# ruiminshen/yolo2-pytorch

Measured on AMD Instinct MI355X. Metric: images/sec (416x416) train+detect, Darknet-19 YOLOv2: value = TRAIN step, batch 64 per GPU (configs[2]) at every N; detect (configs[1]) = roofline.detect_images_per_sec, higher is better.
Workload: dtype f32; 1 GPU; Darknet-19 YOLOv2 20-class train 416x416 batch-64/GPU: fwd + region loss + bwd + SGD (BASELINE configs[2]); classes=20, global_batch=64, parallelism=single GPU, weights=random-init seed 0 (bench_data.randomize)

## Files before the change

yolo2-pytorch_amd/csrc/conv_wgrad.hip:

```cpp
#include <stdlib.h>
#include "common.h"

#ifndef Y2_WGRAD_SPREAD
#define Y2_WGRAD_SPREAD 1
#endif

namespace {

constexpr int NT = 256;
constexpr int KS = 32;

struct WgradArgs {
    const float* x;
    const float* dz;
    float* dw;
    float* partial;
    int B, H, W, Cin, ldx, Cout, ldz, taps;
    int Hi, Wi, stride, pad, KW;
    int M, tiles_i, tiles_j, splits, slabs_per_split;
    unsigned x_bytes, dz_bytes;
    int groups;
    long long gx, gz, gw;
    const int32_t* tile_pix;
    int zW;
};

template <int TI, int WAVES_I, int TJ = 128, bool LIN = false, bool DZRAW = false>
__global__ __launch_bounds__(NT) void conv_wgrad_kernel(const WgradArgs a) {
    constexpr unsigned OOB = 0x80000000u;
    constexpr int WAVES_J = 4 / WAVES_I;
    constexpr int WI = TI / WAVES_I, WJ = TJ / WAVES_J;
    constexpr int IB = WI / 32, JB = WJ / 32;
    constexpr int CA = TI / 4;
    constexpr int RA = NT / CA;
    constexpr int PA = KS / RA;
    constexpr int CB = TJ / 4, RB = NT / CB, PB = KS / RB;
    static_assert(WJ >= 32 && WI >= 32, "a wave owns at least one 32x32 block");
    constexpr int STAGE = KS * TI + KS * TJ;
    typedef __attribute__((address_space(3))) void* lds_ptr_t;
    extern __shared__ __attribute__((aligned(16))) float smem[];

    const int t = threadIdx.x;
    const int lane = t & 63;
    const int wave = __builtin_amdgcn_readfirstlane(t >> 6);
    const int wm = wave / WAVES_J, wn = wave % WAVES_J;
    const int l31 = lane & 31, half = lane >> 5;

    int bid = blockIdx.x;
    int grp = 0;
    if (a.groups > 1) {
        const int per = a.tiles_i * a.tiles_j * a.splits;
        grp = bid / per;
        bid -= grp * per;
    }
    const float* gx_ptr = a.x + (size_t)grp * a.gx;
    const float* gz_ptr = a.dz + (size_t)grp * a.gz;
    float* gw_ptr = a.dw + (size_t)grp * a.gw;
    const int split = bid % a.splits; bid /= a.splits;
    const int tj = bid % a.tiles_j;
    const int ti = bid / a.tiles_j;
    const int i0 = ti * TI, j0 = tj * TJ;
    const int ncols = a.taps * a.Cin;

    const int slab_lo = split * a.slabs_per_split;
    const int nslab_total = (a.M + KS - 1) / KS;
    const int slab_hi = min(nslab_total, slab_lo + a.slabs_per_split);
    const int nk = slab_hi - slab_lo;
    if (nk <= 0) return;

    const int chunk = t % CB;
    const int prow = t / CB;
    const int chunk_a = t % CA;
    const int prow_a = t / CA;
    const int ca = i0 + 4 * chunk_a;
    const bool a_ok = ca < a.Cout;
    const int jb = j0 + 4 * chunk;
    const bool b_ok = jb < ncols;
    const int tap = b_ok ? jb / a.Cin : 0;
    const int ci = b_ok ? jb - tap * a.Cin : 0;
    const int dy = tap / a.KW - a.pad;
    const int dx = tap % a.KW - a.pad;
    int pb[PB], py[PB], px[PB];
    const int q32 = KS / a.W, r32 = KS % a.W;
#pragma unroll
    for (int p = 0; p < PB; ++p) {
        const int m = slab_lo * KS + prow + RB * p;
        pb[p] = m / (a.H * a.W);
        const int idx = m - pb[p] * (a.H * a.W);
        py[p] = idx / a.W;
        px[p] = idx - py[p] * a.W;
    }
    const __amdgpu_buffer_rsrc_t rx = __builtin_amdgcn_make_buffer_rsrc(const_cast<float*>(gx_ptr), 0, a.x_bytes, 0x00020000);
    const __amdgpu_buffer_rsrc_t rz = __builtin_amdgcn_make_buffer_rsrc(const_cast<float*>(gz_ptr), 0, a.dz_bytes, 0x00020000);

    auto issue_slab = [&](int slab, int buf) {
        float* sa = smem + buf * STAGE + wave * 256;
        float* sb = smem + buf * STAGE + KS * TI + wave * 256;
#pragma unroll
        for (int p = 0; p < PA; ++p) {
            const int m = slab * KS + prow_a + RA * p;
            const unsigned va = (m < a.M && a_ok) ? (unsigned)(((size_t)m * a.ldz + ca) * 4) : OOB;
            __builtin_amdgcn_raw_ptr_buffer_load_lds(rz, (lds_ptr_t)(sa + p * RA * TI), 16, (int)va, 0, 0, 0);
        }
#pragma unroll
        for (int p = 0; p < PB; ++p) {
            const int m = slab * KS + prow + RB * p;
            const bool mok = m < a.M;
            const int yi = py[p] * a.stride + dy, xi = px[p] * a.stride + dx;
            const bool in = (unsigned)yi < (unsigned)a.Hi && (unsigned)xi < (unsigned)a.Wi;
            const unsigned vb = (mok && b_ok && in) ? (unsigned)(((size_t)((pb[p] * a.Hi + yi) * a.Wi + xi) * a.ldx + ci) * 4) : OOB;
            __builtin_amdgcn_raw_ptr_buffer_load_lds(rx, (lds_ptr_t)(sb + p * RB * TJ), 16, (int)vb, 0, 0, 0);
        }
#pragma unroll
        for (int p = 0; p < PB; ++p) {
            px[p] += r32; py[p] += q32;
            if (px[p] >= a.W) { px[p] -= a.W; py[p] += 1; }
            while (py[p] >= a.H) { py[p] -= a.H; pb[p] += 1; }
        }
    };

    const int xi = grp >> 2, nu = grp & 3;
    const bool two_i = xi == 1 || xi == 2, two_j = nu == 1 || nu == 2;
    const int i_first = xi == 3 ? 1 : 0, j_first = nu == 3 ? 1 : 0;
    const unsigned pixb = (unsigned)a.ldz * 4u;
    int e_next[PA];
    f32x4 dpx[PA][2][2];
    auto dz_table = [&](int slab) {
#pragma unroll
        for (int p = 0; p < PA; ++p) {
            const int m = slab * KS + prow_a + RA * p;
            e_next[p] = m < a.M ? a.tile_pix[m] : 0x3fffffff;
        }
    };
    auto dz_loads = [&]() {
#pragma unroll
        for (int p = 0; p < PA; ++p) {
            const int e = e_next[p];
            const unsigned pix = (unsigned)e & 0x3fffffffu;
            const bool rowok = a_ok && pix != 0x3fffffffu;
            const bool y1 = (e & 0x40000000) != 0, x1 = e < 0;
            const unsigned base = pix * pixb + (unsigned)ca * 4u;
#pragma unroll
            for (int i = 0; i < 2; ++i)
#pragma unroll
                for (int j = 0; j < 2; ++j) {
                    if ((i == 1 && !two_i) || (j == 1 && !two_j)) continue;
                    const int ii = i_first + i, jj = j_first + j;
                    const bool ok = rowok && (ii == 0 || y1) && (jj == 0 || x1);
                    dpx[p][i][j] = __builtin_bit_cast(f32x4, __builtin_amdgcn_raw_buffer_load_b128(rz, (int)(ok ? base : OOB), (ii * a.zW + jj) * (int)pixb, 0));
                }
        }
    };
    auto dz_store = [&](int buf) {
#pragma unroll
        for (int p = 0; p < PA; ++p) {
            f32x4 sj[2];
#pragma unroll
            for (int j = 0; j < 2; ++j) {
                if (j == 1 && !two_j) continue;
                sj[j] = xi == 0 ? dpx[p][0][j] : (xi == 1 ? dpx[p][0][j] + dpx[p][1][j] : (xi == 2 ? dpx[p][0][j] - dpx[p][1][j] : -dpx[p][0][j]));
            }
            const f32x4 r = nu == 0 ? sj[0] : (nu == 1 ? sj[0] + sj[1] : (nu == 2 ? sj[0] - sj[1] : -sj[0]));
            *reinterpret_cast<f32x4*>(smem + buf * STAGE + p * RA * TI + t * 4) = r;
        }
    };

    f32x16 acc[IB][JB];
#pragma unroll
    for (int i = 0; i < IB; ++i)
#pragma unroll
        for (int j = 0; j < JB; ++j)
#pragma unroll
            for (int r = 0; r < 16; ++r) acc[i][j][r] = 0.f;

    const int fa = wm * WI + l31 + half * TI;
    const int fb = KS * TI + wn * WJ + l31 + half * TJ;

    unsigned nva[PA], nvb[PB];
    if (LIN) {
#pragma unroll
        for (int p = 0; p < PA; ++p) nva[p] = a_ok ? (unsigned)(((size_t)(slab_lo * KS + prow_a + RA * p) * a.ldz + ca) * 4) : OOB;
#pragma unroll
        for (int p = 0; p < PB; ++p) nvb[p] = b_ok ? (unsigned)(((size_t)(slab_lo * KS + prow + RB * p) * a.ldx + ci) * 4) : OOB;
    }
    const unsigned step_a = a_ok ? (unsigned)(KS * a.ldz * 4) : 0u, step_b = b_ok ? (unsigned)(KS * a.ldx * 4) : 0u;
    auto plan_slab = [&](int slab) {
        if (LIN) {
#pragma unroll
            for (int p = 0; p < PA; ++p) nva[p] += step_a;
#pragma unroll
            for (int p = 0; p < PB; ++p) nvb[p] += step_b;
            return;
        }
#pragma unroll
        for (int p = 0; p < PA; ++p) {
            const int m = slab * KS + prow_a + RA * p;
            nva[p] = (m < a.M && a_ok) ? (unsigned)(((size_t)m * a.ldz + ca) * 4) : OOB;
        }
#pragma unroll
        for (int p = 0; p < PB; ++p) {
            const int m = slab * KS + prow + RB * p;
            const bool mok = m < a.M;
            const int yi = py[p] * a.stride + dy, xi = px[p] * a.stride + dx;
            const bool in = (unsigned)yi < (unsigned)a.Hi && (unsigned)xi < (unsigned)a.Wi;
            nvb[p] = (mok && b_ok && in) ? (unsigned)(((size_t)((pb[p] * a.Hi + yi) * a.Wi + xi) * a.ldx + ci) * 4) : OOB;
            px[p] += r32; py[p] += q32;
            if (px[p] >= a.W) { px[p] -= a.W; py[p] += 1; }
            while (py[p] >= a.H) { py[p] -= a.H; pb[p] += 1; }
        }
    };
    auto issue_piece = [&](int buf, int j) {
        if (j < PA) { if (!DZRAW) __builtin_amdgcn_raw_ptr_buffer_load_lds(rz, (lds_ptr_t)(smem + buf * STAGE + wave * 256 + j * RA * TI), 16, (int)nva[j], 0, 0, 0); }
        else __builtin_amdgcn_raw_ptr_buffer_load_lds(rx, (lds_ptr_t)(smem + buf * STAGE + KS * TI + wave * 256 + (j - PA) * RB * TJ), 16, (int)nvb[j - PA], 0, 0, 0);
    };
    auto compute_slab_spread = [&](int buf, int nbuf, int next_slab = 0) {
        const volatile __attribute__((address_space(3))) float* sbuf = (const volatile __attribute__((address_space(3))) float*)(smem + buf * STAGE);
        constexpr int TOTAL = (KS / 2) * IB * JB, NPIECES = PA + PB;
        constexpr int EVERY = (TOTAL / 2) / NPIECES > 0 ? (TOTAL / 2) / NPIECES : 1;
        int cnt = 0;
        float av[2][IB], bv[2][JB];
#pragma unroll
        for (int i = 0; i < IB; ++i) av[0][i] = sbuf[fa + 32 * i];
#pragma unroll
        for (int j = 0; j < JB; ++j) bv[0][j] = sbuf[fb + 32 * j];
#pragma unroll
        for (int s = 0; s < KS / 2; ++s) {
            if (s + 1 < KS / 2) {
#pragma unroll
                for (int i = 0; i < IB; ++i) av[(s + 1) & 1][i] = sbuf[fa + (s + 1) * 2 * TI + 32 * i];
#pragma unroll
                for (int j = 0; j < JB; ++j) bv[(s + 1) & 1][j] = sbuf[fb + (s + 1) * 2 * TJ + 32 * j];
            }
#pragma unroll
            for (int i = 0; i < IB; ++i)
#pragma unroll
                for (int j = 0; j < JB; ++j) {
                    acc[i][j] = __builtin_amdgcn_mfma_f32_32x32x2f32(av[s & 1][i], bv[s & 1][j], acc[i][j], 0, 0, 0);
                    if (cnt % EVERY == 0 && cnt / EVERY < NPIECES) {
                        issue_piece(nbuf, cnt / EVERY);
                        __builtin_amdgcn_sched_barrier(0);
                    }
                    if (DZRAW) {
                        if (cnt == 0) { dz_loads(); __builtin_amdgcn_sched_barrier(0); }
                        if (cnt == 2) { dz_table(next_slab + 1); __builtin_amdgcn_sched_barrier(0); }
                        if (cnt == (TOTAL * 3) / 4) { dz_store(nbuf); __builtin_amdgcn_sched_barrier(0); }
                    }
                    ++cnt;
                }
        }
#pragma unroll
        for (int j = (TOTAL + EVERY - 1) / EVERY; j < NPIECES; ++j) issue_piece(nbuf, j);
    };

    bool blk_ok[IB][JB];
    bool all_ok = true;
#pragma unroll
    for (int i = 0; i < IB; ++i)
#pragma unroll
        for (int j = 0; j < JB; ++j) {
            blk_ok[i][j] = (i0 + wm * WI + i * 32) < a.Cout && (j0 + wn * WJ + j * 32) < ncols;
            all_ok = all_ok && blk_ok[i][j];
        }
    auto compute_slab_checked = [&](int buf) {
        const float* sbuf = smem + buf * STAGE;
#pragma unroll
        for (int s = 0; s < KS / 2; ++s) {
            float av[IB], bv[JB];
#pragma unroll
            for (int i = 0; i < IB; ++i) av[i] = sbuf[fa + s * 2 * TI + 32 * i];
#pragma unroll
            for (int j = 0; j < JB; ++j) bv[j] = sbuf[fb + s * 2 * TJ + 32 * j];
#pragma unroll
            for (int i = 0; i < IB; ++i)
#pragma unroll
                for (int j = 0; j < JB; ++j)
                    if (blk_ok[i][j]) acc[i][j] = __builtin_amdgcn_mfma_f32_32x32x2f32(av[i], bv[j], acc[i][j], 0, 0, 0);
        }
    };

    auto compute_slab = [&](int buf) {
        const float* sbuf = smem + buf * STAGE;
#pragma unroll
        for (int s = 0; s < KS / 2; ++s) {
            float av[IB], bv[JB];
#pragma unroll
            for (int i = 0; i < IB; ++i) av[i] = sbuf[fa + s * 2 * TI + 32 * i];
#pragma unroll
            for (int j = 0; j < JB; ++j) bv[j] = sbuf[fb + s * 2 * TJ + 32 * j];
#pragma unroll
            for (int i = 0; i < IB; ++i)
#pragma unroll
                for (int j = 0; j < JB; ++j)
                    acc[i][j] = __builtin_amdgcn_mfma_f32_32x32x2f32(av[i], bv[j], acc[i][j], 0, 0, 0);
        }
    };

    if (DZRAW) {
        dz_table(slab_lo);
        dz_loads();
        dz_table(slab_lo + 1);
        dz_store(0);
#pragma unroll
        for (int j = PA; j < PA + PB; ++j) issue_piece(0, j);
        for (int ks = 0; ks < nk - 1; ++ks) {
            plan_slab(slab_lo + ks + 1);
            asm volatile("s_waitcnt vmcnt(0)" ::: "memory");
            __syncthreads();
            compute_slab_spread(ks & 1, (ks + 1) & 1, slab_lo + ks + 1);
        }
        asm volatile("s_waitcnt vmcnt(0)" ::: "memory");
        __syncthreads();
        compute_slab((nk - 1) & 1);
    } else {
    issue_slab(slab_lo, 0);
    if (!all_ok) {
        for (int ks = 0; ks < nk - 1; ++ks) {
            asm volatile("s_waitcnt vmcnt(0)" ::: "memory");
            __syncthreads();
            issue_slab(slab_lo + ks + 1, (ks + 1) & 1);
            compute_slab_checked(ks & 1);
        }
        asm volatile("s_waitcnt vmcnt(0)" ::: "memory");
        __syncthreads();
        compute_slab_checked((nk - 1) & 1);
    } else {
        for (int ks = 0; ks < nk - 1; ++ks) {
            if (Y2_WGRAD_SPREAD) plan_slab(slab_lo + ks + 1);
            asm volatile("s_waitcnt vmcnt(0)" ::: "memory");
            __syncthreads();
            if (Y2_WGRAD_SPREAD) {
                compute_slab_spread(ks & 1, (ks + 1) & 1);
            } else {
                issue_slab(slab_lo + ks + 1, (ks + 1) & 1);
                compute_slab(ks & 1);
            }
        }
        asm volatile("s_waitcnt vmcnt(0)" ::: "memory");
        __syncthreads();
        compute_slab((nk - 1) & 1);
    }
    }

#pragma unroll
    for (int jbk = 0; jbk < JB; ++jbk) {
        const int j = j0 + wn * WJ + jbk * 32 + l31;
        if (j >= ncols) continue;
#pragma unroll
        for (int ib = 0; ib < IB; ++ib) {
#pragma unroll
            for (int r = 0; r < 16; ++r) {
                const int co = i0 + wm * WI + ib * 32 + (r & 3) + 8 * (r >> 2) + 4 * half;
                if (co < a.Cout) {
                    if (a.partial != nullptr) {
                        a.partial[((size_t)(grp * a.splits + split) * a.Cout + co) * ncols + j] = acc[ib][jbk][r];
                        continue;
                    }
                    float* dst = gw_ptr + (size_t)co * ncols + j;
                    if (a.splits > 1) atomicAdd(dst, acc[ib][jbk][r]);
                    else *dst = acc[ib][jbk][r];
                }
            }
        }
    }
}

}

static int wgrad_tj(int ncols, int Cout) {
    if (Cout <= 32) return 128;
    const long long p128 = (long long)y2_cdiv(ncols, 128) * 128, p64 = (long long)y2_cdiv(ncols, 64) * 64;
    return (p128 * 100 >= p64 * 115) ? 64 : 128;
}

static int wgrad_splits(long long M, int ncols, int Cout, int groups, int* slabs_per_split) {
    const int TI = Cout <= 32 ? 32 : (Cout <= 64 ? 64 : 128);
    const int TJ = wgrad_tj(ncols, Cout);
    const long long tiles = (long long)y2_cdiv(Cout, TI) * y2_cdiv(ncols, TJ);
    const int slabs = y2_cdiv(M, KS);
    static const int fill_env = getenv("Y2_WGRAD_FILL") != nullptr ? atoi(getenv("Y2_WGRAD_FILL")) : 0;
    const int fill = fill_env > 0 ? fill_env : (TI * TJ >= 128 * 128 ? 2 : (TI * TJ >= 128 * 64 ? 3 : 4));
    int splits = y2_cdiv(fill * Y2_NUM_CU, tiles * groups);
    const int max_splits = slabs / 8 > 0 ? slabs / 8 : 1;
    if (splits > max_splits) splits = max_splits;
    if (splits < 1) splits = 1;
    const int sps = y2_cdiv(slabs, splits);
    if (slabs_per_split != nullptr) *slabs_per_split = sps;
    return y2_cdiv(slabs, sps);
}

int y2_internal_wgrad_needs_zero(long long M, int Cin, int Cout, int groups) {
    return (wgrad_splits(M, Cin, Cout, groups, nullptr) > 1 && !y2_det.on) ? 1 : 0;
}

struct WgradRawDz { const int32_t* tile_pix; int zW, ldz; unsigned long long bytes; };

static int wgrad_impl(const float* x, const float* dz, float* dw, int B, int Hi, int Wi, int Cin, int ldx, int Cout, int ldz,
                      int ksize, int stride, int pad, y2_stream_t stream, int groups, long long gx, long long gz, long long gw, const WgradRawDz* raw = nullptr) {
    if (!x || !dz || !dw || B <= 0 || Hi <= 0 || Wi <= 0 || Cin <= 0 || Cout <= 0) return Y2_EINVAL;
    if (ksize < 1 || ksize > 7 || stride < 1 || pad < 0) return Y2_ENOSUP;
    if (ldx < Cin || ldz < Cout) return Y2_EINVAL;
    if ((Cin & 3) || (ldx & 3) || (Cout & 3) || (ldz & 3) || !y2_aligned16(x) || !y2_aligned16(dz)) return Y2_EALIGN;
    const int H = (Hi + 2 * pad - ksize) / stride + 1, W = (Wi + 2 * pad - ksize) / stride + 1;
    if (H <= 0 || W <= 0) return Y2_EINVAL;
    const long long M = (long long)B * H * W;
    const unsigned long long xb = (unsigned long long)B * Hi * Wi * ldx * 4ull, zb = (unsigned long long)M * ldz * 4ull;
    if (M > 0x3fffffffLL || xb >= 0x7fffffffull || zb >= 0x7fffffffull) return Y2_ENOSUP;
    WgradArgs a;
    a.x = x; a.dz = dz; a.dw = dw;
    a.B = B; a.H = H; a.W = W; a.Cin = Cin; a.ldx = ldx; a.Cout = Cout; a.ldz = ldz; a.taps = ksize * ksize;
    a.Hi = Hi; a.Wi = Wi; a.stride = stride; a.pad = pad; a.KW = ksize;
    a.M = (int)M;
    a.groups = groups; a.gx = gx; a.gz = gz; a.gw = gw;
    const int TI = Cout <= 32 ? 32 : (Cout <= 64 ? 64 : 128);
    a.tiles_i = y2_cdiv(Cout, TI);
    const int TJ = wgrad_tj(a.taps * Cin, Cout);
    a.tiles_j = y2_cdiv(a.taps * Cin, TJ);
    const int tiles = a.tiles_i * a.tiles_j;
    const int slabs = y2_cdiv(M, KS);
    a.splits = wgrad_splits(M, a.taps * Cin, Cout, groups, &a.slabs_per_split);
    a.x_bytes = (unsigned)xb; a.dz_bytes = (unsigned)zb;
    a.tile_pix = nullptr; a.zW = 0;
    if (raw != nullptr) {
        if (groups != 16 || raw->bytes >= 0x7fffffffull || (raw->ldz & 3) || raw->ldz < Cout) return Y2_ENOSUP;
        a.tile_pix = raw->tile_pix; a.zW = raw->zW; a.ldz = raw->ldz; a.dz_bytes = (unsigned)raw->bytes; a.gz = 0;
    }
    a.partial = nullptr;
    const long long wsize = (long long)Cout * a.taps * Cin;
    if (y2_det.on && a.splits > 1) {
        if ((size_t)groups * a.splits * wsize * sizeof(float) > y2_det.bytes) return Y2_EINVAL;
        a.partial = y2_det.ws;
    }
    const long long grid = (long long)tiles * a.splits * groups;
    if (grid > 0x7fffffffLL) return Y2_EINVAL;
    hipStream_t s = y2_s(stream);
    const size_t lds = 2u * (size_t)(KS * TI + KS * TJ) * sizeof(float);
    const bool lin = ksize == 1 && stride == 1 && pad == 0;
#define Y2_WGRAD_LAUNCH_(TI_, WI_, TJ_, LIN_)                                                                             \
    do {                                                                                                                  \
        static Y2LdsAttr attr;                                                                                            \
        if (const int rc_ = attr.ensure(reinterpret_cast<const void*>(conv_wgrad_kernel<TI_, WI_, TJ_, LIN_>))) return rc_;     \
        Y2_LAUNCH(a.groups > 1 ? "conv_wgrad_kernel[grouped]" : "conv_wgrad_kernel", 2.0 * (double)a.M * a.Cout * a.taps * a.Cin * (a.groups > 1 ? a.groups : 1), (conv_wgrad_kernel<TI_, WI_, TJ_, LIN_>), dim3((unsigned)grid), dim3(NT), lds, s, a);                 \
    } while (0)
#define Y2_WGRAD_LAUNCH_RAW(TI_, WI_, TJ_)                                                                                \
    do {                                                                                                                  \
        static Y2LdsAttr attr;                                                                                            \
        if (const int rc_ = attr.ensure(reinterpret_cast<const void*>(conv_wgrad_kernel<TI_, WI_, TJ_, true, true>))) return rc_;     \
        Y2_LAUNCH("conv_wgrad_kernel[grouped,dz]", 2.0 * (double)a.M * a.Cout * a.taps * a.Cin * a.groups, (conv_wgrad_kernel<TI_, WI_, TJ_, true, true>), dim3((unsigned)grid), dim3(NT), lds, s, a);                 \
    } while (0)
#define Y2_WGRAD_LAUNCH(TI_, WI_, TJ_)                                                                                    \
    do {                                                                                                                  \
        if (raw != nullptr) Y2_WGRAD_LAUNCH_RAW(TI_, WI_, TJ_);                                                           \
        else if (lin) Y2_WGRAD_LAUNCH_(TI_, WI_, TJ_, true); else Y2_WGRAD_LAUNCH_(TI_, WI_, TJ_, false);                 \
    } while (0)
    if (TI == 32) Y2_WGRAD_LAUNCH(32, 1, 128);
    else if (TI == 64 && TJ == 64) Y2_WGRAD_LAUNCH(64, 2, 64);
    else if (TI == 64) Y2_WGRAD_LAUNCH(64, 1, 128);
    else if (TJ == 64) Y2_WGRAD_LAUNCH(128, 2, 64);
    else Y2_WGRAD_LAUNCH(128, 2, 128);
#undef Y2_WGRAD_LAUNCH
#undef Y2_WGRAD_LAUNCH_RAW
#undef Y2_WGRAD_LAUNCH_
    Y2_LAUNCH_CHECK();
    if (a.partial != nullptr) {
        for (int g = 0; g < groups; ++g) {
            const int rc = y2_det_reduce_f32(a.partial + (size_t)g * a.splits * wsize, a.splits, wsize, wsize, nullptr, dw + (size_t)g * gw, s);
            if (rc != Y2_OK) return rc;
        }
    }
    return Y2_OK;
}

namespace {

struct W0Args {
    const float* x; const float* dz; float* dw;
    float* partial;
    int B, H, W, Cin, Cout, ldz, rows_total;
};

template <int IB>
__global__ __launch_bounds__(256) void conv0_wgrad_kernel(const W0Args a) {
    __shared__ float red[4][IB * 32 * 33];
    const int t = threadIdx.x, lane = t & 63, wave = t >> 6;
    const int l31 = lane & 31, half = lane >> 5;
    const int K = a.Cin * 9;
    const bool jok = l31 < K;
    const int c = jok ? l31 / 9 : 0;
    const int ky = jok ? (l31 % 9) / 3 : 0, kx = jok ? l31 % 3 : 0;
    f32x16 acc[IB];
#pragma unroll
    for (int i = 0; i < IB; ++i)
#pragma unroll
        for (int r = 0; r < 16; ++r) acc[i][r] = 0.f;
    const int wid = blockIdx.x * 4 + wave, nw = gridDim.x * 4;
    for (int row = wid; row < a.rows_total; row += nw) {
        const int b = row / a.H, y = row - b * a.H;
        const int yy = y + ky - 1;
        const bool yok = jok && (unsigned)yy < (unsigned)a.H;
        const float* xr = a.x + (((size_t)b * a.Cin + c) * a.H + (yok ? yy : 0)) * a.W;
        const float* zr = a.dz + (size_t)row * a.W * a.ldz;
        for (int x0 = 0; x0 < a.W; x0 += 16) {
            float av[IB][8], bv[8];
#pragma unroll
            for (int s = 0; s < 8; ++s) {
                const int px = x0 + 2 * s + half;
                const bool pok = px < a.W;
#pragma unroll
                for (int i = 0; i < IB; ++i) {
                    const int co = i * 32 + l31;
                    av[i][s] = (pok && co < a.Cout) ? zr[(size_t)px * a.ldz + co] : 0.f;
                }
                const int xx = px + kx - 1;
                bv[s] = (pok && yok && (unsigned)xx < (unsigned)a.W) ? xr[xx] : 0.f;
            }
#pragma unroll
            for (int s = 0; s < 8; ++s)
#pragma unroll
                for (int i = 0; i < IB; ++i)
                    acc[i] = __builtin_amdgcn_mfma_f32_32x32x2f32(av[i][s], bv[s], acc[i], 0, 0, 0);
        }
    }
#pragma unroll
    for (int i = 0; i < IB; ++i)
#pragma unroll
        for (int r = 0; r < 16; ++r) {
            const int co = i * 32 + (r & 3) + 8 * (r >> 2) + 4 * half;
            red[wave][co * 33 + l31] = acc[i][r];
        }
    __syncthreads();
    for (int e = t; e < IB * 32 * 32; e += 256) {
        const int co = e >> 5, j = e & 31;
        if (co < a.Cout && j < K) {
            const float v = red[0][co * 33 + j] + red[1][co * 33 + j] + red[2][co * 33 + j] + red[3][co * 33 + j];
            if (a.partial != nullptr) a.partial[(size_t)blockIdx.x * a.Cout * K + (size_t)co * K + j] = v;
            else atomicAdd(a.dw + (size_t)co * K + j, v);
        }
    }
}

}

namespace {

struct W0FArgs {
    const float* x; const float* z; const float* scale; const float* shift; const float* mean; const float* invstd; const float* gamma;
    const float* dy_pool; const double* sums; float* dw;
    float* partial;
    int B, H, W, Cin, Cout, ldz, ldp, pairs_total, has_bn;
    unsigned z_bytes, p_bytes;
    float slope;
    double n;
};

template <int IB>
__global__ __launch_bounds__(256) void conv0_wgrad_fused_kernel(const W0FArgs a) {
    __shared__ float red[4][IB * 32 * 33];
    const int t = threadIdx.x, lane = t & 63, wave = t >> 6;
    const int l31 = lane & 31, half = lane >> 5;
    const int K = a.Cin * 9;
    const bool jok = l31 < K;
    const int c = jok ? l31 / 9 : 0;
    const int ky = jok ? (l31 % 9) / 3 : 0, kx = jok ? l31 % 3 : 0;
    float sc[IB], sh[IB], mu[IB], is[IB], gs[IB], ma[IB], mb[IB];
    bool cok[IB];
#pragma unroll
    for (int i = 0; i < IB; ++i) {
        const int co = i * 32 + l31;
        cok[i] = co < a.Cout;
        const int cc = cok[i] ? co : 0;
        sc[i] = a.scale ? a.scale[cc] : 1.f; sh[i] = a.shift ? a.shift[cc] : 0.f;
        mu[i] = a.has_bn ? a.mean[cc] : 0.f; is[i] = a.has_bn ? a.invstd[cc] : 1.f;
        if (a.has_bn == 1) { gs[i] = a.gamma[cc] * is[i]; ma[i] = (float)(a.sums[cc] / a.n); mb[i] = (float)(a.sums[a.Cout + cc] / a.n); }
        else if (a.has_bn == 2) { gs[i] = a.gamma[cc] * is[i]; ma[i] = 0.f; mb[i] = 0.f; }
        else { gs[i] = 1.f; ma[i] = 0.f; mb[i] = 0.f; }
    }
    f32x16 acc[IB];
#pragma unroll
    for (int i = 0; i < IB; ++i)
#pragma unroll
        for (int r = 0; r < 16; ++r) acc[i][r] = 0.f;
    const int wid = blockIdx.x * 4 + wave, nw = gridDim.x * 4;
    const int Hh = a.H >> 1, Wh = a.W >> 1;
    const __amdgpu_buffer_rsrc_t rz = __builtin_amdgcn_make_buffer_rsrc(const_cast<float*>(a.z), 0, a.z_bytes, 0x00020000);
    const __amdgpu_buffer_rsrc_t rp = __builtin_amdgcn_make_buffer_rsrc(const_cast<float*>(a.dy_pool), 0, a.p_bytes, 0x00020000);
    for (int pair = wid; pair < a.pairs_total; pair += nw) {
        const int b = pair / Hh, r = pair - b * Hh;
        const int y0 = 2 * r;
        const int yy0 = y0 + ky - 1, yy1 = yy0 + 1;
        const bool yok0 = jok && (unsigned)yy0 < (unsigned)a.H, yok1 = jok && (unsigned)yy1 < (unsigned)a.H;
        const float* xr0 = a.x + (((size_t)b * a.Cin + c) * a.H + (yok0 ? yy0 : 0)) * a.W;
        const float* xr1 = a.x + (((size_t)b * a.Cin + c) * a.H + (yok1 ? yy1 : 0)) * a.W;
        const unsigned zrow = (unsigned)(((size_t)(b * a.H + y0) * a.W + half) * a.ldz * 4u) + (unsigned)l31 * 4u;
        const unsigned prow = (unsigned)(((size_t)(b * Hh + r) * Wh) * a.ldp * 4u) + (unsigned)l31 * 4u;
        const unsigned zstep = 2u * (unsigned)a.ldz * 4u, z1off = (unsigned)a.W * (unsigned)a.ldz * 4u, pstep = (unsigned)a.ldp * 4u;
        for (int x0 = 0; x0 < a.W; x0 += 16) {
            float z0[IB][8], z1[IB][8], dp[IB][8], bv0[8], bv1[8];
            const unsigned zb = zrow + (unsigned)x0 * (unsigned)a.ldz * 4u, pb = prow + (unsigned)(x0 >> 1) * pstep;
#pragma unroll
            for (int s = 0; s < 8; ++s) {
                const int px = x0 + 2 * s + half;
#pragma unroll
                for (int i = 0; i < IB; ++i) {
                    z0[i][s] = __builtin_bit_cast(float, __builtin_amdgcn_raw_buffer_load_b32(rz, (int)(zb + i * 128u), (int)(s * zstep), 0));
                    z1[i][s] = __builtin_bit_cast(float, __builtin_amdgcn_raw_buffer_load_b32(rz, (int)(zb + i * 128u), (int)(s * zstep + z1off), 0));
                    dp[i][s] = __builtin_bit_cast(float, __builtin_amdgcn_raw_buffer_load_b32(rp, (int)(pb + i * 128u), (int)(s * pstep), 0));
                }
                const int xx = px + kx - 1;
                const bool xok = (unsigned)xx < (unsigned)a.W;
                bv0[s] = (xok && yok0) ? xr0[xx] : 0.f;
                bv1[s] = (xok && yok1) ? xr1[xx] : 0.f;
            }
#pragma unroll
            for (int s = 0; s < 8; ++s)
#pragma unroll
                for (int i = 0; i < IB; ++i) {
                    const float u0 = z0[i][s] * sc[i] + sh[i], u1 = z1[i][s] * sc[i] + sh[i];
                    const float v0 = u0 > 0.f ? u0 : u0 * a.slope, v1 = u1 > 0.f ? u1 : u1 * a.slope;
                    const float o0 = __shfl_xor(v0, 32), o1 = __shfl_xor(v1, 32);
                    const float q0 = half ? o0 : v0, q1 = half ? v0 : o0, q2 = half ? o1 : v1, q3 = half ? v1 : o1;
                    float best = q0; int arg = 0;
                    if (q1 > best) { best = q1; arg = 1; }
                    if (q2 > best) { best = q2; arg = 2; }
                    if (q3 > best) { best = q3; arg = 3; }
                    const float g0 = (arg == half) ? dp[i][s] : 0.f, g1 = (arg == 2 + half) ? dp[i][s] : 0.f;
                    const float ge0 = g0 * (u0 > 0.f ? 1.f : a.slope), ge1 = g1 * (u1 > 0.f ? 1.f : a.slope);
                    const float zh0 = (z0[i][s] - mu[i]) * is[i], zh1 = (z1[i][s] - mu[i]) * is[i];
                    const bool ok = (x0 + 2 * s + half) < a.W && cok[i];
                    const float d0 = ok ? gs[i] * (ge0 - ma[i] - zh0 * mb[i]) : 0.f;
                    const float d1 = ok ? gs[i] * (ge1 - ma[i] - zh1 * mb[i]) : 0.f;
                    acc[i] = __builtin_amdgcn_mfma_f32_32x32x2f32(d0, bv0[s], acc[i], 0, 0, 0);
                    acc[i] = __builtin_amdgcn_mfma_f32_32x32x2f32(d1, bv1[s], acc[i], 0, 0, 0);
                }
        }
    }
#pragma unroll
    for (int i = 0; i < IB; ++i)
#pragma unroll
        for (int r = 0; r < 16; ++r) {
            const int co = i * 32 + (r & 3) + 8 * (r >> 2) + 4 * half;
            red[wave][co * 33 + l31] = acc[i][r];
        }
    __syncthreads();
    for (int e = t; e < IB * 32 * 32; e += 256) {
        const int co = e >> 5, j = e & 31;
        if (co < a.Cout && j < K) {
            const float v = red[0][co * 33 + j] + red[1][co * 33 + j] + red[2][co * 33 + j] + red[3][co * 33 + j];
            if (a.partial != nullptr) a.partial[(size_t)blockIdx.x * a.Cout * K + (size_t)co * K + j] = v;
            else atomicAdd(a.dw + (size_t)co * K + j, v);
        }
    }
}

}

extern "C" int y2_conv0_wgrad_fused(const float* x_nchw, const float* z, const float* scale, const float* shift, const float* mean, const float* invstd,
                                    const float* gamma, float slope, const float* dy_pool, int ldp, const double* sums, float* dw,
                                    int B, int H, int W, int Cin, int Cout, int ldz, int has_bn, y2_stream_t stream) {
    if (!x_nchw || !z || !dy_pool || !dw || B <= 0 || H <= 0 || W <= 0 || Cout <= 0 || ldz < Cout || ldp < Cout) return Y2_EINVAL;
    if (has_bn < 0 || has_bn > 2 || (has_bn && (!mean || !invstd || !gamma)) || (has_bn == 1 && !sums)) return Y2_EINVAL;
    if ((H & 1) || (W & 1)) return Y2_EINVAL;
    if (Cin < 1 || Cin > 3 || Cout > 64 || (W & 15)) return Y2_ENOSUP;
    const unsigned long long zb = (unsigned long long)B * H * W * ldz * 4ull, pb = (unsigned long long)B * (H / 2) * (W / 2) * ldp * 4ull;
    if (zb >= 0xffff0000ull) return Y2_ENOSUP;
    W0FArgs a;
    a.z_bytes = (unsigned)zb; a.p_bytes = (unsigned)pb;
    a.x = x_nchw; a.z = z; a.scale = scale; a.shift = shift; a.mean = mean; a.invstd = invstd; a.gamma = gamma; a.dy_pool = dy_pool; a.sums = sums; a.dw = dw;
    a.B = B; a.H = H; a.W = W; a.Cin = Cin; a.Cout = Cout; a.ldz = ldz; a.ldp = ldp; a.pairs_total = B * (H / 2); a.has_bn = has_bn; a.slope = slope;
    a.n = (double)B * H * W;
    const int grid = a.pairs_total < 4 * 4 * Y2_NUM_CU ? y2_cdiv(a.pairs_total, 4) : 4 * Y2_NUM_CU;
    a.partial = nullptr;
    if (y2_det.on) {
        if ((size_t)grid * Cout * Cin * 9 * sizeof(float) > y2_det.bytes) return Y2_EINVAL;
        a.partial = y2_det.ws;
    }
    const double flops = 2.0 * (double)B * H * W * 9 * Cin * Cout;
    if (Cout <= 32) Y2_LAUNCH("conv0_wgrad_fused_kernel", flops, (conv0_wgrad_fused_kernel<1>), dim3(grid), dim3(256), 0, y2_s(stream), a);
    else Y2_LAUNCH("conv0_wgrad_fused_kernel", flops, (conv0_wgrad_fused_kernel<2>), dim3(grid), dim3(256), 0, y2_s(stream), a);
    Y2_LAUNCH_CHECK();
    if (a.partial != nullptr) return y2_det_reduce_f32(a.partial, grid, (long long)Cout * Cin * 9, (long long)Cout * Cin * 9, nullptr, dw, y2_s(stream));
    return Y2_OK;
}

extern "C" int y2_conv0_wgrad(const float* x_nchw, const float* dz, float* dw, int B, int H, int W, int Cin, int Cout, int ldz, y2_stream_t stream) {
    if (!x_nchw || !dz || !dw || B <= 0 || H <= 0 || W <= 0 || Cout <= 0 || ldz < Cout) return Y2_EINVAL;
    if (Cin < 1 || Cin > 3 || Cout > 64) return Y2_ENOSUP;
    W0Args a;
    a.x = x_nchw; a.dz = dz; a.dw = dw; a.B = B; a.H = H; a.W = W; a.Cin = Cin; a.Cout = Cout; a.ldz = ldz; a.rows_total = B * H;
    const int grid = a.rows_total < 4 * 4 * Y2_NUM_CU ? y2_cdiv(a.rows_total, 4) : 4 * Y2_NUM_CU;
    a.partial = nullptr;
    if (y2_det.on) {
        if ((size_t)grid * Cout * Cin * 9 * sizeof(float) > y2_det.bytes) return Y2_EINVAL;
        a.partial = y2_det.ws;
    }
    if (Cout <= 32) Y2_LAUNCH("conv0_wgrad_kernel", 2.0 * (double)B * H * W * 9 * Cin * Cout, (conv0_wgrad_kernel<1>), dim3(grid), dim3(256), 0, y2_s(stream), a);
    else Y2_LAUNCH("conv0_wgrad_kernel", 2.0 * (double)B * H * W * 9 * Cin * Cout, (conv0_wgrad_kernel<2>), dim3(grid), dim3(256), 0, y2_s(stream), a);
    Y2_LAUNCH_CHECK();
    if (a.partial != nullptr) return y2_det_reduce_f32(a.partial, grid, (long long)Cout * Cin * 9, (long long)Cout * Cin * 9, nullptr, dw, y2_s(stream));
    return Y2_OK;
}

extern "C" int y2_conv_wgrad_ex(const float* x, const float* dz, float* dw, int B, int Hi, int Wi, int Cin, int ldx, int Cout, int ldz,
                                int ksize, int stride, int pad, y2_stream_t stream) {
    return wgrad_impl(x, dz, dw, B, Hi, Wi, Cin, ldx, Cout, ldz, ksize, stride, pad, stream, 1, 0, 0, 0);
}

int y2_internal_wgrad_grouped(const float* x, const float* dz, float* dw, long long M, int Cin, int Cout, int groups, long long gx, long long gz,
                              long long gw, y2_stream_t stream) {
    if (M <= 0 || M > 0x7fffffffLL || groups < 1) return Y2_EINVAL;
    return wgrad_impl(x, dz, dw, 1, 1, (int)M, Cin, Cin, Cout, Cout, 1, 1, 0, stream, groups, gx, gz, gw);
}

int y2_internal_wgrad_grouped_dz(const float* v, const float* dz_raw, const int32_t* tile_pix, float* dw, long long M, int Cin, int Cout, int ldz, int zW,
                                 unsigned long long dz_bytes, long long gx, long long gw, y2_stream_t stream) {
    if (M <= 0 || M > 0x7fffffffLL || tile_pix == nullptr) return Y2_EINVAL;
    const WgradRawDz raw = {tile_pix, zW, ldz, dz_bytes};
    return wgrad_impl(v, dz_raw, dw, 1, 1, (int)M, Cin, Cin, Cout, Cout, 1, 1, 0, stream, 16, gx, 0, gw, &raw);
}

extern "C" int y2_conv_wgrad(const float* x, const float* dz, float* dw, int B, int H, int W, int Cin, int ldx, int Cout, int ldz,
                             int ksize, y2_stream_t stream) {
    if (ksize != 1 && ksize != 3) return Y2_ENOSUP;
    return y2_conv_wgrad_ex(x, dz, dw, B, H, W, Cin, ldx, Cout, ldz, ksize, 1, (ksize - 1) / 2, stream);
}
```

Measured before the change: 2259 images/sec.

## Add patch-based 3x3 wgrad kernel reusing input halo tiles for small Cin

Adds a specialized weight-gradient kernel for 3x3 stride-1 pad-1 convolutions with Cin=32 (and optionally Cin=64). It loads a spatial patch of input plus halo once into LDS and forms all nine taps from it, instead of going through generic im2col-style per-tap gathers. Global-to-LDS copies are double-buffered and interleaved with MFMA instructions. It also adds an environment override for the split count. This path covers only the early Darknet-19 layer with Cin=32 by default, and it adds new LDS-heavy code plus more atomics or partial-sum reductions.

Result: no change. 2267 images/sec, median of 6 (+0.3%).

```diff
diff --git a/yolo2-pytorch_amd/csrc/conv_wgrad.hip b/yolo2-pytorch_amd/csrc/conv_wgrad.hip
--- a/yolo2-pytorch_amd/csrc/conv_wgrad.hip
+++ b/yolo2-pytorch_amd/csrc/conv_wgrad.hip
@@ -364,8 +364,160 @@
     }
 }
 
-}
-
+struct PatchArgs {
+    const float* x; const float* dz; float* dw; float* partial;
+    int H, W, ldx, Cout, ldz;
+    int YB, SEG, nslab, splits, slabs_per_split;
+    unsigned x_bytes, dz_bytes;
+};
+
+template <int CIN, int TI, int WAVES_I, int SR>
+__global__ __launch_bounds__(192 * WAVES_I) void conv_wgrad_patch_kernel(const PatchArgs a) {
+    constexpr unsigned OOB = 0x80000000u;
+    constexpr int SC = KS / SR, PW = SC + 2, NP = (SR + 2) * PW;
+    constexpr int NW = 3 * WAVES_I;
+    constexpr int WI = TI / WAVES_I, IB = WI / 32, CBLK = CIN / 32, JB = 3 * CBLK;
+    constexpr int PA_TOT = KS * TI / 256, PB_TOT = (NP * CIN + 255) / 256, NPIECE = PA_TOT + PB_TOT;
+    constexpr int PPW = (NPIECE + NW - 1) / NW;
+    constexpr int STAGE = NPIECE * 256;
+    constexpr int LA = TI / 4, LB = CIN / 4;
+    static_assert(CIN % 32 == 0 && WI % 32 == 0 && KS % SR == 0 && (SC & 1) == 0 && PPW <= KS / 2, "shape");
+    typedef __attribute__((address_space(3))) void* lds_ptr_t;
+    extern __shared__ __attribute__((aligned(16))) float smem[];
+
+    const int t = threadIdx.x;
+    const int lane = t & 63;
+    const int wave = __builtin_amdgcn_readfirstlane(t >> 6);
+    const int wm = wave / 3, ky = wave % 3;
+    const int l31 = lane & 31, half = lane >> 5;
+    const int split = blockIdx.x % a.splits;
+    const int i0 = (blockIdx.x / a.splits) * TI;
+    const int ncols = 9 * CIN;
+
+    const int slab_lo = split * a.slabs_per_split;
+    const int slab_hi = min(a.nslab, slab_lo + a.slabs_per_split);
+    const int nk = slab_hi - slab_lo;
+    if (nk <= 0) return;
+
+    const __amdgpu_buffer_rsrc_t rx = __builtin_amdgcn_make_buffer_rsrc(const_cast<float*>(a.x), 0, a.x_bytes, 0x00020000);
+    const __amdgpu_buffer_rsrc_t rz = __builtin_amdgcn_make_buffer_rsrc(const_cast<float*>(a.dz), 0, a.dz_bytes, 0x00020000);
+
+    int rel[PPW], pdy[PPW], pdx[PPW];
+    unsigned voff[PPW];
+#pragma unroll
+    for (int q = 0; q < PPW; ++q) {
+        const int piece = q * NW + wave;
+        if (piece < PA_TOT) {
+            const int k = piece * (256 / TI) + lane / LA, ch = i0 + 4 * (lane % LA);
+            const int r = k / SC, c = k % SC;
+            rel[q] = ((r * a.W + c) * a.ldz + ch) * 4;
+            pdy[q] = ch < a.Cout ? r : (1 << 24);
+            pdx[q] = c;
+        } else {
+            const int p = (piece - PA_TOT) * (256 / CIN) + lane / LB;
+            const int pr = p / PW, pc = p % PW;
+            rel[q] = (((pr - 1) * a.W + (pc - 1)) * a.ldx + 4 * (lane % LB)) * 4;
+            pdy[q] = (piece < NPIECE && p < NP) ? pr - 1 : (1 << 24);
+            pdx[q] = pc - 1;
+        }
+    }
+    int seg = slab_lo % a.SEG, yb, img;
+    { const int u = slab_lo / a.SEG; yb = u % a.YB; img = u / a.YB; }
+    auto plan_slab = [&]() {
+        const int y0 = yb * SR, x0 = seg * SC;
+        const unsigned basepix = (unsigned)((img * a.H + y0) * a.W + x0);
+#pragma unroll
+        for (int q = 0; q < PPW; ++q) {
+            const int piece = q * NW + wave;
+            const unsigned base = basepix * (unsigned)(piece < PA_TOT ? a.ldz : a.ldx) * 4u;
+            const bool ok = (unsigned)(y0 + pdy[q]) < (unsigned)a.H && (unsigned)(x0 + pdx[q]) < (unsigned)a.W;
+            voff[q] = ok ? base + (unsigned)rel[q] : OOB;
+        }
+        if (++seg == a.SEG) { seg = 0; if (++yb == a.YB) { yb = 0; ++img; } }
+    };
+    auto issue_piece = [&](int buf, int q) {
+        const int piece = q * NW + wave;
+        if (piece >= NPIECE) return;
+        const lds_ptr_t dst = (lds_ptr_t)(smem + buf * STAGE + piece * 256);
+        if (piece < PA_TOT) __builtin_amdgcn_raw_ptr_buffer_load_lds(rz, dst, 16, (int)voff[q], 0, 0, 0);
+        else __builtin_amdgcn_raw_ptr_buffer_load_lds(rx, dst, 16, (int)voff[q], 0, 0, 0);
+    };
+
+    f32x16 acc[IB][JB];
+#pragma unroll
+    for (int i = 0; i < IB; ++i)
+#pragma unroll
+        for (int j = 0; j < JB; ++j)
+#pragma unroll
+            for (int r = 0; r < 16; ++r) acc[i][j][r] = 0.f;
+
+    const int fa = wm * WI + l31 + half * TI;
+    const int fb = KS * TI + ky * PW * CIN + l31 + half * CIN;
+    auto compute_slab = [&](int buf, int nbuf, bool fetch) {
+        const volatile __attribute__((address_space(3))) float* sbuf = (const volatile __attribute__((address_space(3))) float*)(smem + buf * STAGE);
+        float av[2][IB], bv[2][JB];
+        auto read_step = [&](int s, int w) {
+            const int pix = ((2 * s) / SC) * PW + (2 * s) % SC;
+#pragma unroll
+            for (int i = 0; i < IB; ++i) av[w][i] = sbuf[fa + s * 2 * TI + 32 * i];
+#pragma unroll
+            for (int j = 0; j < JB; ++j) bv[w][j] = sbuf[fb + (pix + j / CBLK) * CIN + 32 * (j % CBLK)];
+        };
+        read_step(0, 0);
+#pragma unroll
+        for (int s = 0; s < KS / 2; ++s) {
+            if (s + 1 < KS / 2) read_step(s + 1, (s + 1) & 1);
+#pragma unroll
+            for (int i = 0; i < IB; ++i)
+#pragma unroll
+                for (int j = 0; j < JB; ++j) {
+                    acc[i][j] = __builtin_amdgcn_mfma_f32_32x32x2f32(av[s & 1][i], bv[s & 1][j], acc[i][j], 0, 0, 0);
+                    if (i == 0 && j == 0 && s < PPW && fetch) {
+                        issue_piece(nbuf, s);
+                        __builtin_amdgcn_sched_barrier(0);
+                    }
+                }
+        }
+    };
+
+    plan_slab();
+#pragma unroll
+    for (int q = 0; q < PPW; ++q) issue_piece(0, q);
+    for (int ks = 0; ks < nk - 1; ++ks) {
+        plan_slab();
+        asm volatile("s_waitcnt vmcnt(0)" ::: "memory");
+        __syncthreads();
+        compute_slab(ks & 1, (ks + 1) & 1, true);
+    }
+    asm volatile("s_waitcnt vmcnt(0)" ::: "memory");
+    __syncthreads();
+    compute_slab((nk - 1) & 1, 0, false);
+
+#pragma unroll
+    for (int jbk = 0; jbk < JB; ++jbk) {
+        const int j = (ky * 3 + jbk / CBLK) * CIN + (jbk % CBLK) * 32 + l31;
+#pragma unroll
+        for (int ib = 0; ib < IB; ++ib) {
+#pragma unroll
+            for (int r = 0; r < 16; ++r) {
+                const int co = i0 + wm * WI + ib * 32 + (r & 3) + 8 * (r >> 2) + 4 * half;
+                if (co < a.Cout) {
+                    if (a.partial != nullptr) {
+                        a.partial[((size_t)split * a.Cout + co) * ncols + j] = acc[ib][jbk][r];
+                        continue;
+                    }
+                    float* dst = a.dw + (size_t)co * ncols + j;
+                    if (a.splits > 1) atomicAdd(dst, acc[ib][jbk][r]);
+                    else *dst = acc[ib][jbk][r];
+                }
+            }
+        }
+    }
+}
+
+}
+
+static int wgrad_env(const char* name, int dflt);
 static int wgrad_tj(int ncols, int Cout) {
     if (Cout <= 32) return 128;
     const long long p128 = (long long)y2_cdiv(ncols, 128) * 128, p64 = (long long)y2_cdiv(ncols, 64) * 64;
@@ -382,6 +534,8 @@
     int splits = y2_cdiv(fill * Y2_NUM_CU, tiles * groups);
     const int max_splits = slabs / 8 > 0 ? slabs / 8 : 1;
     if (splits > max_splits) splits = max_splits;
+    const int forced = wgrad_env("Y2_WGRAD_SPLITS", 0);
+    if (forced > 0) splits = forced < slabs ? forced : slabs;
     if (splits < 1) splits = 1;
     const int sps = y2_cdiv(slabs, splits);
     if (slabs_per_split != nullptr) *slabs_per_split = sps;
@@ -393,6 +547,59 @@
 }
 
 struct WgradRawDz { const int32_t* tile_pix; int zW, ldz; unsigned long long bytes; };
+
+static int wgrad_env(const char* name, int dflt) {
+    const char* v = getenv(name);
+    return (v != nullptr && *v) ? atoi(v) : dflt;
+}
+
+static int wgrad_patch(const float* x, const float* dz, float* dw, int B, int H, int W, int Cin, int ldx, int Cout, int ldz, unsigned x_bytes, unsigned dz_bytes,
+                       hipStream_t s) {
+    const int mode = wgrad_env("Y2_WGRAD_PATCH", 1);
+    if (mode <= 0 || Cout > 128) return Y2_ENOSUP;
+    if (!(Cin == 32 || (Cin == 64 && wgrad_env("Y2_WGRAD_PATCH64", 0) == 1))) return Y2_ENOSUP;
+    const int TI = Cin == 32 ? 64 : 128, SR = Cin == 32 ? 2 : 4, SC = KS / SR;
+    PatchArgs a;
+    a.x = x; a.dz = dz; a.dw = dw; a.partial = nullptr;
+    a.H = H; a.W = W; a.ldx = ldx; a.Cout = Cout; a.ldz = ldz;
+    a.YB = y2_cdiv(H, SR); a.SEG = y2_cdiv(W, SC);
+    const long long nslab = (long long)B * a.YB * a.SEG;
+    if (nslab > 0x3fffffffLL) return Y2_ENOSUP;
+    a.nslab = (int)nslab;
+    a.x_bytes = x_bytes; a.dz_bytes = dz_bytes;
+    const int tiles = y2_cdiv(Cout, TI);
+    static const int fill_env = getenv("Y2_WGRAD_FILL") != nullptr ? atoi(getenv("Y2_WGRAD_FILL")) : 0;
+    const int forced = wgrad_env("Y2_WGRAD_SPLITS", 0);
+    int splits = forced > 0 ? forced : y2_cdiv((fill_env > 0 ? fill_env : (Cin == 32 ? 4 : 2)) * Y2_NUM_CU, tiles);
+    const int max_splits = a.nslab / 8 > 0 ? a.nslab / 8 : 1;
+    if (forced <= 0 && splits > max_splits) splits = max_splits;
+    if (splits > a.nslab) splits = a.nslab;
+    if (splits < 1) splits = 1;
+    a.slabs_per_split = y2_cdiv(a.nslab, splits);
+    a.splits = y2_cdiv(a.nslab, a.slabs_per_split);
+    const long long wsize = (long long)Cout * 9 * Cin;
+    if (y2_det.on && a.splits > 1) {
+        if ((size_t)a.splits * wsize * sizeof(float) > y2_det.bytes) return Y2_ENOSUP;
+        a.partial = y2_det.ws;
+    }
+    const unsigned grid = (unsigned)(tiles * a.splits);
+    const double flops = 2.0 * (double)B * H * W * Cout * 9 * Cin;
+#define Y2_PATCH_LAUNCH(CIN_, TI_, WI_, SR_)                                                                              \
+    do {                                                                                                                  \
+        constexpr int NP_ = (SR_ + 2) * (KS / SR_ + 2);                                                                   \
+        const size_t lds = 2u * (size_t)(KS * TI_ / 256 + (NP_ * CIN_ + 255) / 256) * 256 * sizeof(float);              \
+        static Y2LdsAttr attr;                                                                                            \
+        if (const int rc_ = attr.ensure(reinterpret_cast<const void*>(conv_wgrad_patch_kernel<CIN_, TI_, WI_, SR_>))) return rc_;     \
+        Y2_LAUNCH("conv_wgrad_patch_kernel", flops, (conv_wgrad_patch_kernel<CIN_, TI_, WI_, SR_>), dim3(grid), dim3(192 * WI_), lds, s, a);     \
+    } while (0)
+    if (Cin == 64) Y2_PATCH_LAUNCH(64, 128, 4, 4);
+    else if (mode == 2) Y2_PATCH_LAUNCH(32, 64, 2, 2);
+    else Y2_PATCH_LAUNCH(32, 64, 1, 2);
+#undef Y2_PATCH_LAUNCH
+    Y2_LAUNCH_CHECK();
+    if (a.partial != nullptr) return y2_det_reduce_f32(a.partial, a.splits, wsize, wsize, nullptr, dw, s);
+    return Y2_OK;
+}
 
 static int wgrad_impl(const float* x, const float* dz, float* dw, int B, int Hi, int Wi, int Cin, int ldx, int Cout, int ldz,
                       int ksize, int stride, int pad, y2_stream_t stream, int groups, long long gx, long long gz, long long gw, const WgradRawDz* raw = nullptr) {
@@ -405,6 +612,10 @@
     const long long M = (long long)B * H * W;
     const unsigned long long xb = (unsigned long long)B * Hi * Wi * ldx * 4ull, zb = (unsigned long long)M * ldz * 4ull;
     if (M > 0x3fffffffLL || xb >= 0x7fffffffull || zb >= 0x7fffffffull) return Y2_ENOSUP;
+    if (groups == 1 && raw == nullptr && ksize == 3 && stride == 1 && pad == 1) {
+        const int rc = wgrad_patch(x, dz, dw, B, Hi, Wi, Cin, ldx, Cout, ldz, (unsigned)xb, (unsigned)zb, y2_s(stream));
+        if (rc != Y2_ENOSUP) return rc;
+    }
     WgradArgs a;
     a.x = x; a.dz = dz; a.dw = dw;
     a.B = B; a.H = H; a.W = W; a.Cin = Cin; a.ldx = ldx; a.Cout = Cout; a.ldz = ldz; a.taps = ksize * ksize;
```
